# hkbharath/MARL-MASS

Hardware: AMD Instinct MI355X
Metric: agent-steps/sec (whole node), MASS CBF shield on, 65536 envs x 8 CAVs (higher is better)
Workload: dtype f64

## Files before the change

marl-mass_amd/csrc/mm_device.h:

```cpp
#pragma once
#include <hip/hip_runtime.h>
#include <stdint.h>

#include "../../include/mm_abi.h"

#define MM_DEV __device__ __forceinline__
#define MMM_FN __device__ __forceinline__
#include "../../include/mm_math.h"
#ifndef MM_QP_NO_CERTIFY
#define MM_QP_CERTIFY
#endif
#include "../../include/mm_qp.h"

namespace mm {

constexpr double kPi = 3.141592653589793;
constexpr double kVehLength = 5.0, kVehWidth = 2.0, kMaxSpeed = 40.0;
constexpr double kTauA = 0.6, kTauDs = 0.2;
constexpr double kLcMaxAcc = 6.0, kLcMinAcc = -12.5;
constexpr double kPerception = 180.0, kStoppingSpeed = 1.6667;
constexpr double kLaneWidth = 4.0;
constexpr double kCbfAccLo = -12.5, kCbfAccHi = 6.0, kAdjBuffer = 2.0134;
constexpr double kSineAmp = 3.25, kSinePuls = 2 * kPi / (2 * 100.0), kSinePhase = kPi / 2;
constexpr double kObstX = 420.0, kObstY = 4.0;
// ... 21 lines not shown
  }
  return a < 0 ? -r : r;
}
MM_DEV double py_mod(double a, double b) {
  double m = fmod_pos(a, b);
  if (m != 0.0) {
    if (m < 0) m += b;
  } else {
    m = 0.0;
  }
  return m;
}
MM_DEV double wrap_to_pi(double x) {
  const double a = x + kPi;
  if (__all(a >= 0.0 && a < 2 * kPi)) return a - kPi;
  return py_mod(a, 2 * kPi) - kPi;
}
MM_DEV double not_zero(double x) {
  return fabs(x) > 1e-2 ? x : (x > 0 ? 1e-2 : -1e-2);
}
MM_DEV double clipd(double x, double a, double b) { return fmin(fmax(x, a), b); }
MM_DEV double div_c(double x, double d, double y) {
  const double q = x * y;
  const double r = fma(-q, d, x);
  return fma(r, y, q);
}
#define MM_DIVC(x, d) ::mm::div_c((x), (d), 1.0 / (d))

MM_DEV void lane_local(int l, double x, double y, double &s, double &r) {
  s = x - lane_sx(l);
  r = y - lane_sy(l);
  if (l == MM_LANE_KB0) r = r - kSineAmp * mmm_sin(kSinePuls * s + kSinePhase);
}
static_assert(kSineAmp * kSinePuls * (1.0 + 0x1p-40) < 0.125, "the sine lane's heading needs the general mmm_atan");
template <bool SINE = false>
MM_DEV double lane_heading_at(int l, double s) {
  if constexpr (SINE) return l == MM_LANE_KB0 ? 0.0 + mmm_atan_small(kSineAmp * kSinePuls * mmm_cos(kSinePuls * s + kSinePhase)) : 0.0;
  else return l == MM_LANE_KB0 ? 0.0 + mmm_atan(kSineAmp * kSinePuls * mmm_cos(kSinePuls * s + kSinePhase)) : 0.0;
}
MM_DEV double lane_distance(int l, double x, double y) {
  double s, r;
  lane_local(l, x, y, s, r);
  return fabs(r) + fmax(s - lane_len(l), 0.0) + fmax(0.0 - s, 0.0);
}
MM_DEV bool lane_on_lane(int l, double x, double y) {
  double s, r;
  lane_local(l, x, y, s, r);
  return fabs(r) <= kLaneWidth / 2 + 0 && (-kVehLength <= s && s < lane_len(l) + kVehLength);
}
MM_DEV bool lane_reachable(int l, double x, double y) {
  if (lane_forbidden(l)) return false;
  double s = x - lane_sx(l), r = y - lane_sy(l);
  return fabs(r) <= 2 * kLaneWidth && (0 <= s && s < lane_len(l) + kVehLength);
}
MM_DEV bool lane_after_end(int l, double x) {
  return (x - lane_sx(l)) > lane_len(l) - kVehLength / 2;
}

template <bool SINE = false>
MM_DEV int closest_lane(double x, double y, double h) {
  const double ang0 = fabs(wrap_to_pi(h - 0.0));
  int best = 0;
  double bd = 0;
#pragma unroll
  for (int l = 0; l < 5; l++) {
    double s = x - lane_sx(l), r = y - lane_sy(l);
    double d = fabs(r) + fmax(s - lane_len(l), 0.0) + fmax(0.0 - s, 0.0) + 1.0 * ang0;
    if (l == 0 || d < bd) { bd = d; best = l; }
  }
  {
    double s = x - 220.0;
    double tail = fmax(s - 100.0, 0.0), head = fmax(0.0 - s, 0.0);
    if (!((0.0 + tail) + head >= bd)) {
      double ph = kSinePuls * s + kSinePhase;
      double sp, cp, lh;
      if constexpr (SINE) {
        mmm_sincos(ph, &sp, &cp);
        lh = 0.0 + mmm_atan_small(kSineAmp * kSinePuls * cp);
      } else {
        sp = mmm_sin(ph); cp = mmm_cos(ph);
        lh = 0.0 + mmm_atan(kSineAmp * kSinePuls * cp);
      }
      double r = (y - 7.25) - kSineAmp * sp;
      double d = fabs(r) + tail + head + 1.0 * fabs(wrap_to_pi(h - lh));
      if (d < bd) { bd = d; best = MM_LANE_KB0; }
    }
  }
  return best;
}
MM_DEV int next_lane(int l, double x, double y) {
  if (l == MM_LANE_AB0 || l == MM_LANE_KB0)
    return lane_distance(MM_LANE_BC0, x, y) <= lane_distance(MM_LANE_BC1, x, y) ? MM_LANE_BC0 : MM_LANE_BC1;
  if (l == MM_LANE_JK0) return MM_LANE_KB0;
  return MM_LANE_CD0;
}

MM_DEV int speed_to_index(double speed) {
  double x = MM_DIVC(speed - 10, 20.0);
  return (int)clipd(rint(x * (5 - 1)), 0, 5 - 1);
}
MM_DEV double index_to_speed(int i) { return 10 + i * (30.0 - 10) / (5 - 1); }

template <bool SINE = false>
MM_DEV double steering_control(double x, double y, double heading, double speed, int tl, double &half_tan) {
  constexpr double KP_HEADING = 1 / kTauDs, KP_LATERAL = 1.0 / 3 * KP_HEADING, PURSUIT_TAU = 0.5 * kTauDs;
  double s, r;
  lane_local(tl, x, y, s, r);
  double lane_next = s + speed * PURSUIT_TAU;
  double lfh = lane_heading_at<SINE>(tl, lane_next);
  double lat_cmd = -KP_LATERAL * r;
  double nz = not_zero(speed);
  double heading_command = mmm_asin(clipd(lat_cmd / nz, -1, 1));
  double heading_ref = lfh + clipd(heading_command, -kPi / 4, kPi / 4);
  double rate = KP_HEADING * wrap_to_pi(heading_ref - heading);
  const double arg = clipd(kVehLength / 2 / nz * rate, -1, 1);
  double w;
  const double steer = mmm_asin_w(arg, &w);
  const bool sat = fabs(steer) > kPi / 3;
  const double ss = sat ? (arg < 0 ? -MMM_SIN_PI3 : MMM_SIN_PI3) : arg;
  const double cs = sat ? MMM_COS_PI3 : w;
  half_tan = 1.0 / 2 * (ss / cs);
  return clipd(steer, -kPi / 3, kPi / 3);
}
MM_DEV double steering_control(double x, double y, double heading, double speed, int tl) {
  double ht;
  return steering_control(x, y, heading, speed, tl, ht);
}

MM_DEV bool has_corner_inside(double c1x, double c1y, double l1, double w1, double a1, double c2x,
                              double c2y, double l2, double w2, double a2) {
  const double lx = l1 / 2, wy = w1 / 2;
  double c = mmm_cos(a1), s = mmm_sin(a1), c2 = mmm_cos(a2), s2 = mmm_sin(a2);
  const double px[9] = {0, -lx, lx, 0, 0, -lx, -lx, lx, lx};
  const double py[9] = {0, 0, 0, -wy, wy, -wy, wy, -wy, wy};
  bool any = false;
#pragma unroll
  for (int k = 0; k < 9; k++) {
    double rx = c * px[k] + (-s) * py[k], ry = s * px[k] + c * py[k];
    double dx = (c1x + rx) - c2x, dy = (c1y + ry) - c2y;
    double ru0 = c2 * dx + (-s2) * dy, ru1 = s2 * dx + c2 * dy;
// ... 37 lines not shown
```

marl-mass_amd/csrc/mm_kernels.hip:

```cpp
#include <hip/hip_runtime.h>
#include <math.h>
#include <stdio.h>
#include <string.h>

#include <type_traits>

#include "mm_device.h"
#include "mm_div.h"
#include "mm_handle.h"
#define MM_COUNTS_FN __host__ __device__ inline
#include "../../include/mm_counts.h"
#include "../../include/mm_policy_wide.h"

using namespace mm;

struct DevCfg {
  int env_kind, shield, nsub, T, action_masking, auto_reset, obs_f64, N, E, debug_flags, n_hdv;
  double dt, collision_reward, high_speed_reward, headway_cost, headway_time, merging_lane_cost;
  double rs_lo, rs_hi, eta, tau;
  double inv_dt, rs_span, rs_ispan, rs_span2, rs_ispan2;
  int agent_reward;
  int steer_vel;
  int *err;
  int traffic_density, mixed_traffic, num_cav;
// ... 41 lines not shown
};

#ifndef MM_TU
#define MM_TU 0
#endif

#ifdef MM_STAMPS
#define MM_STAMP_WAVES (1 << 16)
__device__ unsigned long long g_stamps_w[MM_STAMP_WAVES * 16];
__device__ unsigned long long g_stamps_s[4096 * 8];
#define SSTAMP(k)                                                                        \
  do {                                                                                   \
    unsigned long long _t = __builtin_amdgcn_s_memtime();                                \
    if ((threadIdx.x & 63) == (k)) _t_acc += _t - _t_last;                               \
    _t_last = __builtin_amdgcn_s_memtime();                                              \
  } while (0)
#define SCOUNT(k) do { if ((threadIdx.x & 63) == (k)) _t_acc += 1; } while (0)
#define STAMP(k)                                                                         \
  do {                                                                                   \
    unsigned long long _t = __builtin_amdgcn_s_memtime();                                \
    if ((threadIdx.x & 63) == (k)) _t_acc += _t - _t_last;                               \
    _t_last = __builtin_amdgcn_s_memtime();                                              \
  } while (0)
enum { MM_CS_UPFRONT_CYCLES = 16,
       MM_CS_UPFRONT,
       MM_CS_LAZY_B,
       MM_CS_FALLBACK,
       MM_CS_PRIOR_HELD,
       MM_CS_PRIOR_LIFTED,
       MM_CS_LAZY_A,
       MM_CS_FIRST_B,
       MM_CS_NEAR,
       MM_CS_NEAR_ANY,
       MM_CS_PRECHECK };
__device__ unsigned long long g_stamps_c[MM_STAMP_WAVES * 16];
#define CAND_COUNT(k, cond)                                                                                  \
  do {                                                                                                       \
    const unsigned long long _m = __ballot(cond);                                                            \
    if ((threadIdx.x & 63) == (k)) _t_acc += (unsigned long long)__popcll(_m) + (_m ? 1ull << 32 : 0ull);    \
  } while (0)
#else
#define STAMP(k) do {} while (0)
#define SSTAMP(k) do {} while (0)
#define SCOUNT(k) do {} while (0)
#define CAND_COUNT(k, cond) do {} while (0)
#endif

template <int KIND> constexpr bool kIdm = KIND == MM_ENV_HDV_V1;

struct Veh {
  double x, y, h, v, tspeed;
  double act_steer, act_acc, safe_steer, safe_acc, gvx;
  double h1x, h1vx, h2x, h2vx;
  double sang;
  int lane, tlane, sidx, crashed, hl, flags, hist_len;
  int kind;
  bool present;
};

MM_DEV int lane_id() { return threadIdx.x & 63; }
MM_DEV double shfl_d(double v, int src) { return __shfl(v, src, 64); }
MM_DEV int shfl_i(int v, int src) { return __shfl(v, src, 64); }

template <int CTRL>
MM_DEV int dpp_perm(int v) {
  static_assert((CTRL >= 0x00 && CTRL <= 0xFF) || (CTRL >= 0x121 && CTRL <= 0x12F) || CTRL == 0x140 || CTRL == 0x141,
                "only controls without invalid source lanes: quad_perm, row_ror, row_mirror, row_half_mirror");
// ... 3 lines not shown
MM_DEV int dppx_i(int v) {
  static_assert(M >= 1 && M <= 15, "xor mask within a 16-lane DPP row");
  if constexpr (M == 1) return dpp_perm<0xB1>(v);
  else if constexpr (M == 2) return dpp_perm<0x4E>(v);
  else if constexpr (M == 3) return dpp_perm<0x1B>(v);
  else if constexpr (M == 7) return dpp_perm<0x141>(v);
  else if constexpr (M == 8) return dpp_perm<0x128>(v);
  else if constexpr (M == 15) return dpp_perm<0x140>(v);
  else if constexpr (M < 7) return dppx_i<7>(dppx_i<7 - M>(v));
  else if constexpr (M < 12) return dppx_i<8>(dppx_i<M - 8>(v));
  else return dppx_i<15>(dppx_i<15 - M>(v));
}
template <int M>
MM_DEV double dppx_d(double v) {
  long long b = __double_as_longlong(v);
  int lo = dppx_i<M>((int)(unsigned)(b & 0xFFFFFFFFll)), hi = dppx_i<M>((int)(b >> 32));
  return __longlong_as_double(((long long)hi << 32) | (unsigned)lo);
}
template <int M, int G, class F>
MM_DEV void for_partners_impl(F &f) {
  if constexpr (M < G) {
    f(std::integral_constant<int, M>{});
    for_partners_impl<M + 1, G>(f);
  }
}
template <int G, class F>
MM_DEV void for_partners(F f) { for_partners_impl<1, G>(f); }

template <int G> constexpr bool kPow2 = (G & (G - 1)) == 0;
#ifndef MM_ROUNDS_LITE
#define MM_ROUNDS_LITE 1
#endif
constexpr bool kRoundsLite = MM_ROUNDS_LITE != 0;
#ifndef MM_VETO_PRIOR
#define MM_VETO_PRIOR 1
#endif
constexpr bool kVetoPrior = MM_VETO_PRIOR != 0;
template <int M, int G>
MM_DEV int pidx(int a) {
  if constexpr (kPow2<G>) return a ^ M;
  else return a + M >= G ? a + M - G : a + M;
}
template <int G>
MM_DEV int pidx_rt(int a, int m) {
  if constexpr (kPow2<G>) return a ^ m;
  else return a + m >= G ? a + m - G : a + m;
}
template <int M, int G>
MM_DEV int plane(int lane, int a) {
  if constexpr (kPow2<G>) return lane ^ M;
  else return lane - a + pidx<M, G>(a);
}
template <int G>
MM_DEV int plane_rt(int lane, int a, int m) {
  if constexpr (kPow2<G>) return lane ^ m;
  else return lane - a + pidx_rt<G>(a, m);
}
template <int M, int G>
MM_DEV int px_i(int v, int a) {
  if constexpr (kPow2<G>) return dppx_i<M>(v);
  else return shfl_i(v, plane<M, G>(lane_id(), a));
}
template <int M, int G>
MM_DEV double px_d(double v, int a) {
  if constexpr (kPow2<G>) return dppx_d<M>(v);
  else return shfl_d(v, plane<M, G>(lane_id(), a));
// ... 96 lines not shown
  if (action == 2 || action == 0) {
    int cand = v.tlane;
    if (lane_road(v.tlane) == 1) cand = (action == 2) ? MM_LANE_BC1 : MM_LANE_BC0;
    if (lane_reachable(cand, v.x, v.y)) v.tlane = cand;
  }
}

MM_DEV void clip_actions(Veh &v, bool lc_vehicle, double &st_t) {
  if (v.crashed) { v.act_steer = 0; st_t = 0; v.act_acc = -1.0 * v.v; }
  if (v.v > kMaxSpeed) v.act_acc = fmin(v.act_acc, 1.0 * (kMaxSpeed - v.v));
  else if (v.v < -kMaxSpeed) v.act_acc = fmax(v.act_acc, 1.0 * (kMaxSpeed - v.v));
  if (lc_vehicle) v.act_acc = clipd(v.act_acc, kLcMinAcc, kLcMaxAcc);
}

MM_DEV int corner_flags(double x, double y, double sh, double ch, int lane) {
  double cx = x + (kCornerLen * mmm_cos_sum(MMM_CORNER_SIN, MMM_CORNER_COS, sh, ch));
  double cyL = y - (kCornerLen * mmm_sin_sum(MMM_CORNER_SIN, MMM_CORNER_COS, sh, ch)) + 0.01;
  double cyR = y - (kCornerLen * mmm_sin_sum(-MMM_CORNER_SIN, MMM_CORNER_COS, sh, ch)) + 0.01;
  double s = cx - lane_sx(lane);
  double off = (lane == MM_LANE_KB0) ? kSineAmp * mmm_sin(kSinePuls * s + kSinePhase) : 0.0;
  bool lon = (-kVehLength <= s && s < lane_len(lane) + kVehLength);
  double rL = cyL - lane_sy(lane), rR = cyR - lane_sy(lane);
  if (lane == MM_LANE_KB0) { rL = rL - off; rR = rR - off; }
  return (!(fabs(rL) <= kLaneWidth / 2 + 0 && lon) ? 1 : 0) | (!(fabs(rR) <= kLaneWidth / 2 + 0 && lon) ? 2 : 0);
}
MM_DEV int pose_code(int lane, int nl, int off) { return lane | nl << 3 | off << 6; }

struct Cand {
  double x, y, h, gvx, cpsi, spsi;
  int lane;
  int pk;
};
template <int KIND, bool SHIELDED, bool CORNERS = SHIELDED, bool GENERAL = true, bool SINE = false>
MM_DEV Cand predict(const Veh &v, double steer, double st_t, double sh, double ch, double dt, bool sv = false) {
  Cand c;
  double ht = st_t, sb, cb;
  if constexpr (GENERAL) {
    if (__any(sv || st_t != st_t)) {
      double s2, c2;
      mmm_sincos(sv ? v.sang : steer, &s2, &c2);
      if (sv || st_t != st_t) ht = 1.0 / 2 * (s2 / c2);
    }
  }
  mmm_slip_sincos(ht, &sb, &cb);
  double vx = v.v * mmm_cos_sum(sh, ch, sb, cb), vy = v.v * mmm_sin_sum(sh, ch, sb, cb);
  c.x = v.x + vx * dt;
  c.y = v.y + vy * dt;
  const double d_heading = MM_DIVC(v.v * sb, 2.5);
  c.h = v.h + (sv ? d_heading : d_heading * dt);
  mmm_sincos(c.h, &c.spsi, &c.cpsi);
  c.gvx = (KIND == MM_ENV_V1) ? mmm_cos_sum(c.spsi, c.cpsi, sb, cb) : 0.0;
  c.lane = closest_lane<SINE>(c.x, c.y, c.h);
  c.pk = c.lane;
  if (SHIELDED) c.pk = pose_code(c.lane, next_lane(c.lane, c.x, c.y), CORNERS ? corner_flags(c.x, c.y, c.spsi, c.cpsi, c.lane) : 0);
  return c;
}

MM_DEV int adj_pair(int l1, int l2) {
  return (l1 == MM_LANE_BC0 && l2 == MM_LANE_BC1) ? -1 : ((l1 == MM_LANE_BC1 && l2 == MM_LANE_BC0) ? 1 : 0);
}
MM_DEV int adj_lane(int l1, int nl1, int l2) {
  const int f = adj_pair(l1, l2);
  return f != 0 ? f : adj_pair(nl1, l2);
}
MM_DEV unsigned adj_row(int l1) { return l1 == MM_LANE_BC0 ? (3u << (2 * MM_LANE_BC1)) : (l1 == MM_LANE_BC1 ? (1u << (2 * MM_LANE_BC0)) : 0u); }
MM_DEV unsigned adj_col(int l2) { return l2 == MM_LANE_BC1 ? (3u << (2 * MM_LANE_BC0)) : (l2 == MM_LANE_BC0 ? (1u << (2 * MM_LANE_BC1)) : 0u); }

struct QpTrace {
  double rows, a, h0, h1, h2, h3, d, margin;
};

MM_DEV void init_vehicle(Veh &v) {
  v.lane = closest_lane(v.x, v.y, v.h);
  v.tlane = v.lane;
  v.act_steer = v.act_acc = 0;
  v.safe_steer = v.safe_acc = 0;
  if (v.kind == 2) {
    v.sidx = 0;
    v.tspeed = v.v;
    v.gvx = py_mod((v.x + v.y) * kPi, 1.0);
  } else {
    v.sidx = speed_to_index(v.v);
    v.tspeed = index_to_speed(v.sidx);
    v.gvx = __builtin_nan("");
  }
// ... 322 lines not shown
  s.h2 = -s.v_min + s.u0;
  s.hls_lona = s.px_lona + s.q_lona;
  s.hls_lonr = s.px_lonr + s.q_lonr;
  s.can_abort_lc = (pk_self >> 6) == 0;
  return s;
}
template <bool MASS>
MM_DEV double slot_gu(double vx, double acc, double g, double dt) {
  double u = vx + acc * dt;
  u = u > 0 ? u : 0;
  return (MASS ? g * dt : 1 * dt) * u;
}
struct ShieldRows { double g2u2, g4u4, h0, h3; };
template <bool PRE>
MM_DEV ShieldRows shield_rows(const DevCfg &c, const ShieldStatic &s, const Neigh &nb) {
  const double dt = c.dt;
  ShieldRows r;
  if (PRE) {
    r.g2u2 = nb.has_ol ? nb.ol_gu : 0.0;
    r.g4u4 = nb.has_oa ? nb.oa_gu : 0.0;
  } else {
    double u2 = 0, u4 = 0;
    if (nb.has_ol) { u2 = nb.ol_vx + nb.ol_acc * dt; u2 = u2 > 0 ? u2 : 0; }
    if (nb.has_oa) { u4 = nb.oa_vx + nb.oa_acc * dt; u4 = u4 > 0 ? u4 : 0; }
    r.g2u2 = s.g2 * u2;
    r.g4u4 = s.g4 * u4;
  }
  const double g0u0 = s.g0 * s.u0;
  r.h0 = s.base0 + (-g0u0 + r.g2u2);
  r.h3 = __builtin_nan("");
  if (s.cadj) r.h3 = s.base3 + (-g0u0 + r.g4u4);
  return r;
}
MM_DEV double qp_exact(const ShieldStatic &s, const ShieldRows &r) {
  const double hc = (s.cadj && r.h3 < r.h0) ? r.h3 : r.h0;
  double d;
  if (s.g0 > 0) d = fmin(0.0, hc / s.g0);
  else if (s.g0 < 0) d = fmax(0.0, hc / s.g0);
  else d = 0.0;
  return fmin(fmax(d, -s.h2), s.h1);
}
template <bool MASS>
MM_DEV ShieldOut shield_post(const DevCfg &c, const Veh &v, const ShieldStatic &s, const ShieldRows &r, double d, bool optimal, bool check) {
  const double dt = c.dt, eta = c.eta;
  ShieldOut o;
  o.optimal = optimal;
  o.bounds = check && ((s.u0 + d) - 0.001 > s.v_max || (s.u0 + d) + 0.001 < s.v_min);
  double us0 = s.u0 + d;
  {
    const double hls_lon = s.px_lon + s.q_lon;
    const double hlds_lon = s.px_lon + ((-s.g0) * us0 + r.g2u2) + s.q_lon;
    o.lon_safe = hls_lon >= -1e-6;
    o.lon_invariant = (hlds_lon + (eta - 1) * hls_lon) >= -1e-6;
    o.hw_num = s.px_lon - kVehLength; o.hw_den = s.evx;
  }
  const double hlds_lona = s.px_lona + ((-s.g0) * us0 + r.g4u4) + s.q_lona;
  const double hlds_lonr = s.px_lonr + (s.g0 * us0 + (-s.g6) * s.u6) + s.q_lonr;
  const double inv_lona = hlds_lona + (eta - 1) * s.hls_lona, inv_lonr = hlds_lonr + (eta - 1) * s.hls_lonr;
  const bool lc_allowed = ((s.hls_lona >= 0) && inv_lona >= 0) && ((s.hls_lonr >= 0) && inv_lonr >= 0);
  int fl = v.flags & MM_FLAG_COLLABORATE_ADJ;
  if (s.cadj) fl |= MM_FLAG_IS_COLLABORATING;
  bool veto;
  if (!MASS) {
    veto = !lc_allowed;
  } else {
    veto = s.can_abort_lc && !lc_allowed;
// ... 455 lines not shown
#endif
constexpr int step_min_waves(bool ipm = false) { return SHIELD == MM_SHIELD_NONE ? (G >= MM_NONE_WIDE_G ? 2 : (MIXED ? MM_GENERAL_NONE_WAVES : MM_NONE_WAVES)) : (ipm ? (G >= 6 ? MM_IPM_WIDE_WAVES : (MIXED ? MM_IPM_WAVES : MM_IPM_CAV_WAVES)) : MM_MIN_WAVES); }
template <int G, int KIND, int SHIELD, bool MIXED, bool IPM = false, bool TRACE = false, bool SPLIT = false>
#ifndef MM_STEP_BLOCK
#define MM_STEP_BLOCK 64
#endif
__global__ __launch_bounds__(MM_STEP_BLOCK, (SPLIT ? MM_SPLIT_WAVES : step_min_waves<G, SHIELD, MIXED>(IPM))) void step_kernel(DevCfg c, DevState st, const int32_t *__restrict__ actions,
                                                   MMStepOut out, double *metrics, SweepBuf sb, int kb, PoseBuf pb) {
  constexpr bool IDM = kIdm<KIND>;
  constexpr bool LC = (KIND == MM_ENV_V1) || IDM;
  constexpr bool SHIELDED = LC && (SHIELD != MM_SHIELD_NONE);
  static_assert(!IDM || (MIXED && SHIELD == MM_SHIELD_NONE && !IPM && !SPLIT), "hdv-v1: general unshielded kernels only");
  constexpr bool MASS = (SHIELD == MM_SHIELD_MASS);
  static_assert(!IPM || SHIELDED, "the IPM mode lives in shielded kernels");
  static_assert(!SPLIT || IPM, "the split form exists for the interior-point kernels");
#ifdef MM_SERIAL_ALL
  constexpr bool kSerialOnly = true || IPM;
#else
#ifdef MM_SERIAL_MASS
  constexpr bool kSerialOnly = MIXED || MASS || IPM;
#else
  constexpr bool kSerialOnly = MIXED;
#endif
#endif
  constexpr bool kSine = SHIELDED && !SPLIT && !MIXED && !IPM && !kSerialOnly && kPow2<G> && G <= 8;
#ifndef MM_CARRY_POSE
#define MM_CARRY_POSE 1
#endif
  constexpr bool kCarry = kSine && MM_CARRY_POSE != 0;
#ifndef MM_PRIMARY_PRIOR
#define MM_PRIMARY_PRIOR 1
#endif
  constexpr bool kPrimary = kSine && !TRACE && kVetoPrior && MM_PRIMARY_PRIOR != 0;
  static_assert(kPow2<G> || MM_STEP_BLOCK == 64, "rotation layouts: one wave per workgroup");
  const long long gtid = (long long)blockIdx.x * blockDim.x + threadIdx.x;
  constexpr int kTail = kPow2<G> ? 64 : (64 / G) * G;
  const bool tail = lane_id() >= kTail;
  const int gb = kPow2<G> ? (lane_id() & ~(G - 1)) : (tail ? kTail - G : lane_id() - lane_id() % G);
  const int a = kPow2<G> ? (int)(gtid % G) : lane_id() - gb;
  const long long e = kPow2<G> ? gtid / G : (tail ? (long long)st.E : (gtid >> 6) * (64 / G) + lane_id() / G);
  const bool valid = e < st.E && a < st.N;
  const long long i = e * st.N + a;
  const long long A = st.A;
  const double dt = c.dt;

#ifdef MM_STAMPS
  unsigned long long _t_last = __builtin_amdgcn_s_memtime(), _t_acc = 0;
#endif
  Veh v;
  const bool sv = MIXED && KIND == MM_ENV_V1 && c.steer_vel != 0;
  int steps = 0, time = 0, n_merge = 0, episode = 0;
  int car_code = 0;
  long long car_kx = 0, car_ky = 0, car_kh = 0;
  double car_s = 0.0, car_c = 1.0;
  if constexpr (kCarry) {
    if (valid) {
      car_kx = __double_as_longlong(pb.F[PB_KX * A + i]); car_ky = __double_as_longlong(pb.F[PB_KY * A + i]);
      car_kh = __double_as_longlong(pb.F[PB_KH * A + i]);
      car_s = pb.F[PB_SIN * A + i]; car_c = pb.F[PB_COS * A + i]; car_code = pb.code[i];
    }
  }
  load_veh(st, i, valid, v, sv);
  if (e < st.E) {
    steps = st.I[MM_E_STEPS * st.E + e]; time = st.I[MM_E_TIME * st.E + e];
  }
  if (!MIXED && v.kind == 2) v.kind = 1;
// ... 142 lines not shown
        }
        if constexpr (MIXED) { STAMP(4); }
        if (acting && timer_due) v.gvx = 0;
        int tl_post = acting ? (lc_branch ? my_tl : (mobil_go ? side : my_tl)) : v.tlane;
        for (int round = 0; round <= st.N; round++) {
          bool hit = false;
          for_partners<G>([&](auto mc) {
            constexpr int m = decltype(mc)::value;
            const int p = pidx<m, G>(a);
            const int pk = px_i<m, G>(rank | tl_pre << 4 | tl_post << 8, a);
            const int p_tl = ((pk & 15) < rank) ? ((pk >> 8) & 7) : ((pk >> 4) & 7);
            hit = hit || (((abort_mask >> p) & 1u) && p_tl == my_tl);
          });
          const int nxt = (acting && lc_branch) ? ((same_road && hit) ? v.lane : my_tl) : tl_post;
          const bool changed = nxt != tl_post;
          tl_post = nxt;
          if (!__any(changed)) break;
        }
        if constexpr (MIXED) { STAMP(5); }
        if (acting) {
          v.tlane = tl_post;
          v.act_acc = clipd(acc_f0, -6.0, 6.0);
        }
      }
      if (head && live && (!hdv || !v.crashed)) steer_lane(v, sv && !hdv, st_t);
      if (head && hdv && live) v.gvx += dt;
    }
    bool first_B = false;
    if constexpr (kPrimary) {
      static_assert(!MIXED && !SPLIT, "kPrimary: no HDVs, no steer_vel, every launch a whole step");
      first_B = (c.debug_flags & 1) == 0 && live && v.hist_len >= 2 && (v.tlane != v.lane || v.crashed) && !(v.flags & MM_FLAG_IS_LC_SAFE);
      if (live) {
        const int tl_1 = v.tlane + (first_B ? v.lane - v.tlane : 0);
        const double steer = steering_control<kSine>(v.x, v.y, v.h, v.v, tl_1, st_t);
        v.act_steer = clipd(steer, -kPi / 3, kPi / 3);
        const double steer_1 = v.act_steer, st_t_1 = st_t;
        clip_actions(v, LC, st_t);
        if (first_B) { v.act_steer = steer_1; st_t = st_t_1; }
      }
    } else {
      if (live && head) clip_actions(v, LC && !hdv, st_t);
    }
    STAMP(1);
    Cand cA;
    memset(&cA, 0, sizeof cA);
    const bool shield_on = SHIELDED && live && !hdv && v.hist_len >= 2;
    if (live && head) cA = predict<KIND, SHIELDED, MASS, MIXED, kSine>(v, v.act_steer, st_t, spsi, cpsi, dt, sv && !hdv);
    auto park = [&](auto base_c, const Cand &cc, double steer) {
      constexpr int base = decltype(base_c)::value;
      if constexpr (SHIELDED) {
        s_cold[base + 0][tid] = cc.x; s_cold[base + 1][tid] = cc.y; s_cold[base + 2][tid] = cc.h;
        cold_i(base + 3, tid) = cc.pk; s_cold[base + 4][tid] = cc.cpsi; s_cold[base + 5][tid] = steer;
        s_cold[base + 6][tid] = cc.gvx; s_cold[base + 7][tid] = cc.spsi;
      }
    };
    auto park_at = [&](int base, const Cand &cc, double steer) {
      s_cold[base + 0][tid] = cc.x; s_cold[base + 1][tid] = cc.y; s_cold[base + 2][tid] = cc.h;
      cold_i(base + 3, tid) = cc.pk; s_cold[base + 4][tid] = cc.cpsi; s_cold[base + 5][tid] = steer;
      s_cold[base + 6][tid] = cc.gvx; s_cold[base + 7][tid] = cc.spsi;
    };
    if constexpr (kPrimary) park_at(first_B ? (int)C_B : (int)C_A, cA, v.act_steer);
    else if (head) park(std::integral_constant<int, C_A>{}, cA, v.act_steer);
    STAMP(2);
    const bool needB = SHIELDED && shield_on && (v.tlane != v.lane || v.crashed || sv);
    bool haveB = first_B, haveA = !first_B;
    (void)haveA;
    auto make_other = [&]() {
      if constexpr (kPrimary) {
        const bool mk_A = !haveA;
        if (mk_A || (needB && !haveB)) {
          double t_o;
          const int tl_o = v.lane + (mk_A ? v.tlane - v.lane : 0);
          double steer_o = steering_control<kSine>(v.x, v.y, v.h, v.v, tl_o, t_o);
          if (mk_A) {
            steer_o = clipd(steer_o, -kPi / 3, kPi / 3);
            if (v.crashed) { steer_o = 0; t_o = 0; }
          }
          park_at(mk_A ? (int)C_A : (int)C_B, predict<KIND, true, MASS, MIXED, kSine>(v, steer_o, t_o, spsi, cpsi, dt, false), steer_o);
          haveA = true; haveB = haveB || !mk_A;
        }
// ... 242 lines not shown
                const unsigned long long fm = __ballot(fin);
                ready = ready && (!ol_dyn || ((fm >> src_ol) & 1ull)) && (!oa_dyn || ((fm >> src_oa) & 1ull));
              }
              if (__any(ready)) {
                if (ready) {
                  if (MASS) { if (ol_dyn) nb.ol_gu = da; if (oa_dyn) nb.oa_gu = db; }
                  const ShieldRows rw = shield_rows<true>(c, ss, nb);
                  const int rows = ss.cadj ? 4 : 3;
                  if ((qc_meta & 7) == rows && __double_as_longlong(qc_h0) == __double_as_longlong(rw.h0) &&
                      __double_as_longlong(qc_h3) == __double_as_longlong(rw.h3)) {
                    q.x0 = qc_d; late = true; late_opt = (qc_meta & 8) != 0;
                  } else {
                    qc_h0 = rw.h0; qc_h3 = rw.h3;
                    sing = false;
                    int stop = mm_qp_start(&q, ss.g0, rw.h0, ss.h1, ss.h2, rw.h3, rows) != 0 ? 0 : 2;
                    if (!stop) stop = mm_qp_top(&q, &rs);
                    run = stop == 0;
                    if (stop) { late = true; late_opt = stop == 1; }
                  }
                }
              }
              const bool any_run = __any(run);
              if (any_run) {
                if (run) sing = mm_qp_bottom(&q, &rs) == 0;
              }
              more = any_run || __any(!fin);
            }
            if (shield_on) so = shield_post<MASS>(c, v, ss, shield_rows<true>(c, ss, nb), qc_d, (qc_meta & 8) != 0, true);
          } else {
          if constexpr (MASS && kRoundsLite) {
            const bool slow_lc = (v.hl == 2 || v.hl == 0) && v.v < kStoppingSpeed;
            ShieldRows rr;
            double d_cur = 0.0;
            for (int round = 0; round <= st.N; round++) {
#if defined(MM_STAMPS) && defined(MM_COUNT_ROUNDS)
              if ((threadIdx.x & 63) == 13) _t_acc += 1;
#endif
              const double gu_cur = slot_gu<true>(h1vx_mine, acc_cur, mine_gvx, dt);
              const double da = shfl_d(gu_cur, src_ol), db = shfl_d(gu_cur, src_oa);
              if (ol_dyn) nb.ol_gu = da;
              if (oa_dyn) nb.oa_gu = db;
              rr = shield_rows<true>(c, ss, nb);
              d_cur = qp_exact(ss, rr);
              double acc_next = v.act_acc;
              if (shield_on) {
                if (slow_lc) acc_next = shield_post<true>(c, v, ss, rr, d_cur, true, false).acc;
                else acc_next = div_c((ss.u0 + d_cur) - ss.evx, dt, c.inv_dt);
              }
              const bool changed = __double_as_longlong(acc_next) != __double_as_longlong(acc_cur);
              acc_cur = acc_next;
              if (!__any(changed)) break;
            }
            so = shield_post<true>(c, v, ss, rr, d_cur, true, false);
          } else {
          for (int round = 0; round <= st.N; round++) {
            if (MASS) {
              const double gu_cur = slot_gu<true>(h1vx_mine, acc_cur, mine_gvx, dt);
              const double da = shfl_d(gu_cur, src_ol), db = shfl_d(gu_cur, src_oa);
              if (ol_dyn) nb.ol_gu = da;
              if (oa_dyn) nb.oa_gu = db;
            }
            so = shield_dyn<MASS, true, false>(c, v, ss, nb, shield_on);
            const double acc_next = shield_on ? so.acc : v.act_acc;
            const bool changed = __double_as_longlong(acc_next) != __double_as_longlong(acc_cur);
            acc_cur = acc_next;
            if (!MASS || !__any(changed)) break;
          }
          }
          }
          if (TRACE && shield_on) trace_status(out.trace + (long long)k * MM_T_COUNT * A + i, A, so);
          STAMP(4);
          const bool want_B = shield_on && so.veto && needB;
          CAND_COUNT(MM_CS_LAZY_B, want_B && !haveB);
          if constexpr (kPrimary) {
            CAND_COUNT(MM_CS_LAZY_A, !want_B && !haveA);
            if (want_B ? !haveB : !haveA) make_other();
          } else {
            if (want_B) make_B();
          }
          STAMP(5);
          const bool flip = want_B != use_B;
          use_B = want_B;
          if (!__any(flip)) break;
        }
        serial = __any(irregular);
        if (!serial && shield_on) {
// ... 101 lines not shown
          const bool mine = has && a == ai && shield_on;
          ShieldOut s1 = shield_eval<MASS, true, IPM>(c, v, cpsi, pk_self, nb, mine);
          if (hss_collab) s1.flags |= MM_FLAG_IS_COLLABORATING;
          if (IPM && mine && s1.bounds) atomicOr(c.err, MM_LATCH_QP_BOUNDS);
          if (mine) {
            new_acc = s1.acc; veto = s1.veto; new_flags = s1.flags; qt = s1.qt;
            if (TRACE) trace_status(out.trace + (long long)k * MM_T_COUNT * A + i, A, s1);
            use_B = veto && needB;
            const Cand cc = chosen(use_B);
            double nv = v.v + new_acc * dt;
            nv = nv > 0 ? nv : 0;
            wx = cc.x; wy = cc.y; wh = cc.h; wg = cc.gvx; wacc = new_acc; wvx = nv * cc.cpsi;
            whx = s_cold[C_H1X][tid]; whvx = s_cold[C_H1VX][tid]; wpk = cc.pk;
            wgu = slot_gu<MASS>(whvx, MASS ? wacc : kCbfAccLo, wg, dt);
          }
        }
        if (MIXED && hdv && twin_shift != 0 && w_stepped) s_cold[C_H1X][tid] = whx;
      }
     }
    }
    STAMP(6);
    CAND_COUNT(MM_CS_PRIOR_HELD, st_prior && use_B);
    CAND_COUNT(MM_CS_PRIOR_LIFTED, st_prior && !use_B);
    if (SPLIT && SHIELDED && out.trace && live && tail && !shield_on) {
      out.trace[(long long)k * MM_T_COUNT * A + i + MM_T_QP_ROWS * A] = 0;
    }
    if (!SPLIT && SHIELDED && TRACE && live) {
      double *t = out.trace + (long long)k * MM_T_COUNT * A + i;
      t[MM_T_QP_ROWS * A] = qt.rows; t[MM_T_QP_A * A] = qt.a;
      t[MM_T_QP_H0 * A] = qt.h0; t[MM_T_QP_H1 * A] = qt.h1; t[MM_T_QP_H2 * A] = qt.h2;
      t[MM_T_QP_H3 * A] = qt.h3; t[MM_T_QP_D * A] = qt.d; t[MM_T_LC_MARGIN * A] = qt.margin;
    }
    if (tail) {
    if (live) {
      const Cand cc = chosen(use_B);
      const double acc = (SHIELDED && shield_on) ? new_acc : v.act_acc;
      double nv = v.v + acc * dt;
      nv = nv > 0 ? nv : 0;
      if (SHIELDED && shield_on) {
        if (veto) v.tlane = v.lane;
        v.flags = new_flags;
      }
      v.x = cc.x; v.y = cc.y; v.h = cc.h; v.v = nv; v.lane = cc.lane;
      if (LC) {
        if (!hdv) {
          double steer_nom = v.act_steer;
          if constexpr (SHIELDED) steer_nom = s_cold[C_A + 5][tid];
          s_cold[C_SSTEER][tid] = (SHIELDED && shield_on && veto && haveB) ? s_cold[C_B + 5][tid] : steer_nom;
          s_cold[C_SACC][tid] = acc; v.gvx = cc.gvx;
          if constexpr (kRoomy) s_cold[C_GVX][tid] = cc.gvx;
          if (sv) v.sang += s_cold[C_SSTEER][tid] * dt;
        }
        s_cold[C_H2X][tid] = s_cold[C_H1X][tid]; s_cold[C_H2VX][tid] = s_cold[C_H1VX][tid];
        s_cold[C_H1X][tid] = v.x; s_cold[C_H1VX][tid] = v.v * cc.cpsi;
        if (v.hist_len < 2) v.hist_len++;
      }
      if constexpr (kRoomy) s_cold[C_CPSI][tid] = cc.cpsi;
      else cpsi = cc.cpsi;
      spsi = cc.spsi;
      if (SHIELDED) pk_self = cc.pk;
    }

    STAMP(7);
    unsigned need = 0;
#ifdef MM_STAMPS
    bool near_any = false;
// ... 1468 lines not shown
extern "C" int32_t mm_debug_read_sweep_stamps(unsigned long long *out8, int32_t reset) {
  static unsigned long long host[4096 * 8];
  hipError_t rc = hipMemcpyFromSymbol(host, HIP_SYMBOL(g_stamps_s), sizeof host);
  for (int k = 0; k < 8; k++) out8[k] = 0;
  for (int w = 0; w < 4096; w++)
    for (int k = 0; k < 8; k++) out8[k] += host[w * 8 + k];
  if (rc == hipSuccess && reset) {
    memset(host, 0, sizeof host);
    rc = hipMemcpyToSymbol(HIP_SYMBOL(g_stamps_s), host, sizeof host);
  }
  return rc == hipSuccess ? MM_OK : MM_ERR_DEVICE;
}
extern "C" int32_t mm_debug_read_stamps(unsigned long long *out16, int32_t reset) {
  static unsigned long long *host = nullptr;
  if (!host) host = (unsigned long long *)malloc(sizeof(unsigned long long) * MM_STAMP_WAVES * 16);
  hipError_t rc = hipMemcpyFromSymbol(host, HIP_SYMBOL(g_stamps_w), sizeof(unsigned long long) * MM_STAMP_WAVES * 16);
  for (int k = 0; k < 16; k++) out16[k] = 0;
  for (long long w = 0; w < MM_STAMP_WAVES; w++)
    for (int k = 0; k < 16; k++) out16[k] += host[w * 16 + k];
  if (rc == hipSuccess && reset) {
    memset(host, 0, sizeof(unsigned long long) * MM_STAMP_WAVES * 16);
    rc = hipMemcpyToSymbol(HIP_SYMBOL(g_stamps_w), host, sizeof(unsigned long long) * MM_STAMP_WAVES * 16);
  }
  return rc == hipSuccess ? MM_OK : MM_ERR_DEVICE;
}
extern "C" int32_t mm_debug_read_cand_stamps(unsigned long long *out32, int32_t reset) {
  static unsigned long long *host = nullptr;
  if (!host) host = (unsigned long long *)malloc(sizeof(unsigned long long) * MM_STAMP_WAVES * 16);
  hipError_t rc = hipMemcpyFromSymbol(host, HIP_SYMBOL(g_stamps_c), sizeof(unsigned long long) * MM_STAMP_WAVES * 16);
  for (int k = 0; k < 32; k++) out32[k] = 0;
  for (long long w = 0; w < MM_STAMP_WAVES; w++)
    for (int k = 0; k < 16; k++) {
      const unsigned long long x = host[w * 16 + k];
      if (k == MM_CS_UPFRONT_CYCLES - 16) { out32[k] += x; continue; }
      out32[k] += x & 0xFFFFFFFFull;
      out32[16 + k] += x >> 32;
    }
  if (rc == hipSuccess && reset) {
    memset(host, 0, sizeof(unsigned long long) * MM_STAMP_WAVES * 16);
    rc = hipMemcpyToSymbol(HIP_SYMBOL(g_stamps_c), host, sizeof(unsigned long long) * MM_STAMP_WAVES * 16);
  }
  return rc == hipSuccess ? MM_OK : MM_ERR_DEVICE;
}
#endif
#endif
```

Measured before the change: 2.463 billion.

## Seed shield fixed-point rounds with prior acceleration and add optional sine-carry path

```diff
diff --git a/marl-mass_amd/csrc/mm_device.h b/marl-mass_amd/csrc/mm_device.h
--- a/marl-mass_amd/csrc/mm_device.h
+++ b/marl-mass_amd/csrc/mm_device.h
@@ -77,6 +77,14 @@
   r = y - lane_sy(l);
   if (l == MM_LANE_KB0) r = r - kSineAmp * mmm_sin(kSinePuls * s + kSinePhase);
 }
+MM_DEV void lane_local_carried(int l, double x, double y, double car, double &s, double &r) {
+  s = x - lane_sx(l);
+  r = y - lane_sy(l);
+  const bool kb = l == MM_LANE_KB0;
+  double sn = car;
+  if (__any(kb && car != car)) sn = (car != car) ? mmm_sin(kSinePuls * s + kSinePhase) : car;
+  if (kb) r = r - kSineAmp * sn;
+}
 static_assert(kSineAmp * kSinePuls * (1.0 + 0x1p-40) < 0.125, "the sine lane's heading needs the general mmm_atan");
 template <bool SINE = false>
 MM_DEV double lane_heading_at(int l, double s) {
@@ -103,7 +111,8 @@
 }
 
 template <bool SINE = false>
-MM_DEV int closest_lane(double x, double y, double h) {
+MM_DEV int closest_lane(double x, double y, double h, double *sine_out = nullptr) {
+  if (sine_out) *sine_out = __builtin_nan("");
   const double ang0 = fabs(wrap_to_pi(h - 0.0));
   int best = 0;
   double bd = 0;
@@ -126,6 +135,7 @@
         sp = mmm_sin(ph); cp = mmm_cos(ph);
         lh = 0.0 + mmm_atan(kSineAmp * kSinePuls * cp);
       }
+      if (sine_out) *sine_out = sp;
       double r = (y - 7.25) - kSineAmp * sp;
       double d = fabs(r) + tail + head + 1.0 * fabs(wrap_to_pi(h - lh));
       if (d < bd) { bd = d; best = MM_LANE_KB0; }
@@ -146,11 +156,12 @@
 }
 MM_DEV double index_to_speed(int i) { return 10 + i * (30.0 - 10) / (5 - 1); }
 
-template <bool SINE = false>
-MM_DEV double steering_control(double x, double y, double heading, double speed, int tl, double &half_tan) {
+template <bool SINE = false, bool CARRIED = false>
+MM_DEV double steering_control(double x, double y, double heading, double speed, int tl, double &half_tan, double car = 0.0) {
   constexpr double KP_HEADING = 1 / kTauDs, KP_LATERAL = 1.0 / 3 * KP_HEADING, PURSUIT_TAU = 0.5 * kTauDs;
   double s, r;
-  lane_local(tl, x, y, s, r);
+  if constexpr (CARRIED) lane_local_carried(tl, x, y, car, s, r);
+  else lane_local(tl, x, y, s, r);
   double lane_next = s + speed * PURSUIT_TAU;
   double lfh = lane_heading_at<SINE>(tl, lane_next);
   double lat_cmd = -KP_LATERAL * r;
diff --git a/marl-mass_amd/csrc/mm_kernels.hip b/marl-mass_amd/csrc/mm_kernels.hip
--- a/marl-mass_amd/csrc/mm_kernels.hip
+++ b/marl-mass_amd/csrc/mm_kernels.hip
@@ -97,7 +97,14 @@
        MM_CS_FIRST_B,
        MM_CS_NEAR,
        MM_CS_NEAR_ANY,
-       MM_CS_PRECHECK };
+       MM_CS_PRECHECK,
+       MM_CS_ROUND_CYCLES,
+       MM_CS_ROUNDS,
+       MM_CS_PASSES,
+       MM_CS_SEED_ACTIVE,
+       MM_CS_DIAG_CYCLES };
+static_assert(MM_CS_DIAG_CYCLES == 31, "sixteen slots: lanes 16 .. 31");
+constexpr bool mm_cs_is_cycles(int slot) { return slot == MM_CS_UPFRONT_CYCLES || slot == MM_CS_ROUND_CYCLES || slot == MM_CS_DIAG_CYCLES; }
 __device__ unsigned long long g_stamps_c[MM_STAMP_WAVES * 16];
 #define CAND_COUNT(k, cond)                                                                                  \
   do {                                                                                                       \
@@ -167,6 +174,10 @@
 #define MM_ROUNDS_LITE 1
 #endif
 constexpr bool kRoundsLite = MM_ROUNDS_LITE != 0;
+#ifndef MM_ROUNDS_PRIOR
+#define MM_ROUNDS_PRIOR 1
+#endif
+constexpr bool kRoundsPrior = MM_ROUNDS_PRIOR != 0;
 #ifndef MM_VETO_PRIOR
 #define MM_VETO_PRIOR 1
 #endif
@@ -329,7 +340,7 @@
   int pk;
 };
 template <int KIND, bool SHIELDED, bool CORNERS = SHIELDED, bool GENERAL = true, bool SINE = false>
-MM_DEV Cand predict(const Veh &v, double steer, double st_t, double sh, double ch, double dt, bool sv = false) {
+MM_DEV Cand predict(const Veh &v, double steer, double st_t, double sh, double ch, double dt, bool sv = false, double *sine_out = nullptr) {
   Cand c;
   double ht = st_t, sb, cb;
   if constexpr (GENERAL) {
@@ -347,7 +358,7 @@
   c.h = v.h + (sv ? d_heading : d_heading * dt);
   mmm_sincos(c.h, &c.spsi, &c.cpsi);
   c.gvx = (KIND == MM_ENV_V1) ? mmm_cos_sum(c.spsi, c.cpsi, sb, cb) : 0.0;
-  c.lane = closest_lane<SINE>(c.x, c.y, c.h);
+  c.lane = closest_lane<SINE>(c.x, c.y, c.h, sine_out);
   c.pk = c.lane;
   if (SHIELDED) c.pk = pose_code(c.lane, next_lane(c.lane, c.x, c.y), CORNERS ? corner_flags(c.x, c.y, c.spsi, c.cpsi, c.lane) : 0);
   return c;
@@ -736,6 +747,7 @@
   if (s.cadj) r.h3 = s.base3 + (-g0u0 + r.g4u4);
   return r;
 }
+MM_DEV double rounds_seed(const DevCfg &c, const ShieldStatic &s) { return div_c(s.u0 - s.evx, c.dt, c.inv_dt); }
 MM_DEV double qp_exact(const ShieldStatic &s, const ShieldRows &r) {
   const double hc = (s.cadj && r.h3 < r.h0) ? r.h3 : r.h0;
   double d;
@@ -1257,6 +1269,12 @@
 #define MM_PRIMARY_PRIOR 1
 #endif
   constexpr bool kPrimary = kSine && !TRACE && kVetoPrior && MM_PRIMARY_PRIOR != 0;
+#ifndef MM_SINE_CARRY
+#define MM_SINE_CARRY 0
+#endif
+  constexpr bool kSineCarry = kPrimary && MM_SINE_CARRY != 0;
+  double car_sn = __builtin_nan("");
+  (void)car_sn;
   static_assert(kPow2<G> || MM_STEP_BLOCK == 64, "rotation layouts: one wave per workgroup");
   const long long gtid = (long long)blockIdx.x * blockDim.x + threadIdx.x;
   constexpr int kTail = kPow2<G> ? 64 : (64 / G) * G;
@@ -1465,7 +1483,7 @@
       first_B = (c.debug_flags & 1) == 0 && live && v.hist_len >= 2 && (v.tlane != v.lane || v.crashed) && !(v.flags & MM_FLAG_IS_LC_SAFE);
       if (live) {
         const int tl_1 = v.tlane + (first_B ? v.lane - v.tlane : 0);
-        const double steer = steering_control<kSine>(v.x, v.y, v.h, v.v, tl_1, st_t);
+        const double steer = steering_control<kSine, kSineCarry>(v.x, v.y, v.h, v.v, tl_1, st_t, car_sn);
         v.act_steer = clipd(steer, -kPi / 3, kPi / 3);
         const double steer_1 = v.act_steer, st_t_1 = st_t;
         clip_actions(v, LC, st_t);
@@ -1478,7 +1496,8 @@
     Cand cA;
     memset(&cA, 0, sizeof cA);
     const bool shield_on = SHIELDED && live && !hdv && v.hist_len >= 2;
-    if (live && head) cA = predict<KIND, SHIELDED, MASS, MIXED, kSine>(v, v.act_steer, st_t, spsi, cpsi, dt, sv && !hdv);
+    if constexpr (kSineCarry) car_sn = __builtin_nan("");
+    if (live && head) cA = predict<KIND, SHIELDED, MASS, MIXED, kSine>(v, v.act_steer, st_t, spsi, cpsi, dt, sv && !hdv, kSineCarry ? &car_sn : nullptr);
     auto park = [&](auto base_c, const Cand &cc, double steer) {
       constexpr int base = decltype(base_c)::value;
       if constexpr (SHIELDED) {
@@ -1787,10 +1806,29 @@
             const bool slow_lc = (v.hl == 2 || v.hl == 0) && v.v < kStoppingSpeed;
             ShieldRows rr;
             double d_cur = 0.0;
+            if constexpr (kRoundsPrior) {
+              if (shield_on) acc_cur = rounds_seed(c, ss);
+            }
+#ifdef MM_STAMPS
+            {
+              STAMP(4);
+              const double a_seed = shield_on ? rounds_seed(c, ss) : v.act_acc;
+              const double gu_seed = slot_gu<true>(h1vx_mine, a_seed, mine_gvx, dt);
+              const double da = shfl_d(gu_seed, src_ol), db = shfl_d(gu_seed, src_oa);
+              Neigh ns = nb;
+              if (ol_dyn) ns.ol_gu = da;
+              if (oa_dyn) ns.oa_gu = db;
+              const double d_seed = qp_exact(ss, shield_rows<true>(c, ss, ns));
+              CAND_COUNT(MM_CS_PASSES, shield_on);
+              CAND_COUNT(MM_CS_SEED_ACTIVE, shield_on && d_seed != 0.0);
+              STAMP(MM_CS_DIAG_CYCLES);
+            }
+#endif
             for (int round = 0; round <= st.N; round++) {
 #if defined(MM_STAMPS) && defined(MM_COUNT_ROUNDS)
               if ((threadIdx.x & 63) == 13) _t_acc += 1;
 #endif
+              CAND_COUNT(MM_CS_ROUNDS, shield_on);
               const double gu_cur = slot_gu<true>(h1vx_mine, acc_cur, mine_gvx, dt);
               const double da = shfl_d(gu_cur, src_ol), db = shfl_d(gu_cur, src_oa);
               if (ol_dyn) nb.ol_gu = da;
@@ -1807,6 +1845,7 @@
               if (!__any(changed)) break;
             }
             so = shield_post<true>(c, v, ss, rr, d_cur, true, false);
+            STAMP(MM_CS_ROUND_CYCLES);
           } else {
           for (int round = 0; round <= st.N; round++) {
             if (MASS) {
@@ -1974,6 +2013,9 @@
       t[MM_T_QP_H3 * A] = qt.h3; t[MM_T_QP_D * A] = qt.d; t[MM_T_LC_MARGIN * A] = qt.margin;
     }
     if (tail) {
+    if constexpr (kSineCarry) {
+      if (!(live && use_B == first_B)) car_sn = __builtin_nan("");
+    }
     if (live) {
       const Cand cc = chosen(use_B);
       const double acc = (SHIELDED && shield_on) ? new_acc : v.act_acc;
@@ -3508,7 +3550,7 @@
   for (long long w = 0; w < MM_STAMP_WAVES; w++)
     for (int k = 0; k < 16; k++) {
       const unsigned long long x = host[w * 16 + k];
-      if (k == MM_CS_UPFRONT_CYCLES - 16) { out32[k] += x; continue; }
+      if (mm_cs_is_cycles(k + 16)) { out32[k] += x; continue; }
       out32[k] += x & 0xFFFFFFFFull;
       out32[16 + k] += x >> 32;
     }
```

Result: faster. 2.491 billion, median of 6 (+1.1%).
